# madeleineudell/LowRankModels.jl

Measured on AMD Instinct MI355X. Metric: observed-entry updates/sec, higher is better.
Workload: dtype f64

## Files before the change

lowrankmodels.jl_amd/csrc/glrm_cached.hpp:

```cpp
#pragma once

#include <hip/hip_runtime.h>

#include <algorithm>

#include "glrm_device.hpp"
#include "glrm_engine.hpp"
#include "glrm_launch.hpp"
#include "glrm_sweep.hpp"

namespace glrm {

struct CachedArgs {
  int64_t nseg;
  const int64_t* ptr;
  const int32_t* idx;
  const double* vals;
  double* own;
  int64_t own_offset;
  const double* other;
  double* alpha;
  const glrm_loss* losses;
  const glrm_reg* regs;
  int reg_single;
  int k;
  double fixed_alpha;
  double min_stepsize;
  int32_t* trials;
  int32_t* accepts;
  int cap;
  const int32_t* seglist;
  int64_t seg_lo, seg_hi;
  int vecreg;
};

__device__ __forceinline__ int64_t cached_segment(const CachedArgs& a, int64_t slot) {
  if (slot >= a.nseg) return -1;
  if (!a.seglist) return slot;
  const int64_t seg = a.seglist[slot];
  return (seg < a.seg_lo || seg >= a.seg_hi) ? -1 : seg;
}

__device__ __forceinline__ double cached_wide(double v) { return v; }
__device__ __forceinline__ double cached_wide(float v) {
  double d;
  asm volatile("v_cvt_f64_f32 %0, %1" : "=v"(d) : "v"(v));
  return d;
}

template <int G, int R, int LOSS, int MAXT, bool GRAD, int WAVES = 1, class ST = double>
__device__ __forceinline__ double reg_pass(const CachedArgs& a, const typename Pair<ST>::type (&y)[MAXT][R / 2], const ST (&av)[MAXT], const int (&cc)[MAXT],
                                           const Vec<G, R>& xv, Vec<G, R>& g, int len, int gi, const LossDesc& segloss) {
  constexpr int NG = (64 / G) * WAVES, LM = loss_mode(LOSS);
  constexpr bool TRIG = loss_trig(LOSS);
  double J = 0.0;
  if (GRAD) {
#pragma unroll
    for (int i = 0; i < R / 2; ++i) g.v[i] = make_double2(0.0, 0.0);
  }
#pragma unroll
  for (int t = 0; t < MAXT; ++t) {
    if (t * NG + (gi & ~(64 / G - 1)) < len) {
      double dot = 0.0;
#pragma unroll
      for (int i = 0; i < R / 2; ++i) {
        dot = fma(xv.v[i].x, cached_wide(y[t][i].x), dot);
        dot = fma(xv.v[i].y, cached_wide(y[t][i].y), dot);
      }
      dot = group_sum<G>(dot);
      double L, dL;
      if constexpr (LOSS == LOSS_QUAD_UNIFORM) {
        const double d = dot - (double)av[t];
        L = segloss.scale * (d * d);
        dL = 2 * d * segloss.scale;
      } else if constexpr (LM == LOSS_SEGMENT) {
        loss_both<GRAD, TRIG>(segloss, dot, (double)av[t], L, dL);
      } else {
        const LossDesc lo = load_loss(a.losses, cc[t]);
        loss_both<GRAD, TRIG>(lo, dot, (double)av[t], L, dL);
      }
      if (!(t * NG + gi < len)) {
        L = 0.0;
        dL = 0.0;
      }
      J += L;
      if (GRAD) {
#pragma unroll
        for (int i = 0; i < R / 2; ++i) {
          g.v[i].x = fma(dL, cached_wide(y[t][i].x), g.v[i].x);
          g.v[i].y = fma(dL, cached_wide(y[t][i].y), g.v[i].y);
        }
      }
    }
  }
  J = across_groups_sum<G>(J);
  if (GRAD) {
#pragma unroll
    for (int i = 0; i < R / 2; ++i) {
      g.v[i].x = across_groups_sum<G>(g.v[i].x);
      g.v[i].y = across_groups_sum<G>(g.v[i].y);
    }
  }
  return J;
}

template <int G, int R, int WAVES, bool GRAD>
__device__ __forceinline__ double row_combine(double J, Vec<G, R>& g, double* red, int wave, int lane) {
  constexpr int KP = G * R, STRIDE = KP + 2;
  if constexpr (WAVES == 1) return J;
  const int j = lane % G;
  __syncthreads();
  if (lane < G) {
    if (GRAD) {
#pragma unroll
      for (int i = 0; i < R / 2; ++i) *reinterpret_cast<double2*>(&red[wave * STRIDE + i * 2 * G + 2 * j]) = g.v[i];
    }
    if (lane == 0) red[wave * STRIDE + KP] = J;
  }
  __syncthreads();
  double Js = 0.0;
  if (GRAD) {
#pragma unroll
    for (int i = 0; i < R / 2; ++i) g.v[i] = make_double2(0.0, 0.0);
  }
  for (int w = 0; w < WAVES; ++w) {
    Js += red[w * STRIDE + KP];
    if (GRAD) {
#pragma unroll
      for (int i = 0; i < R / 2; ++i) {
        const double2 p = *reinterpret_cast<const double2*>(&red[w * STRIDE + i * 2 * G + 2 * j]);
        g.v[i].x += p.x;
        g.v[i].y += p.y;
      }
    }
  }
  return Js;
}

template <class ST, int G, int R>
__device__ __forceinline__ void round_trial(Vec<G, R>& xn) {
  if constexpr (sizeof(ST) == 4) {
#pragma unroll
    for (int i = 0; i < R / 2; ++i) xn.v[i] = make_double2(stored<ST>(xn.v[i].x), stored<ST>(xn.v[i].y));
  }
}

template <int G, int R, int LOSS, int MAXT, int WAVES, bool VR = false, class ST = double>
__global__ void __launch_bounds__(WAVES * 64) regcached_sweep_kernel(const CachedArgs a) {
  using P = typename Pair<ST>::type;
  constexpr int KP = G * R, NG = (64 / G) * WAVES;
  __shared__ __attribute__((aligned(16))) double red[WAVES == 1 ? 2 : WAVES * (KP + 2)];
  const int lane = threadIdx.x & 63, wave = threadIdx.x >> 6;
  const int64_t seg = cached_segment(a, blockIdx.x);
  if (seg < 0) return;
  const int j = lane % G, gi = wave * (64 / G) + lane / G;
  const int64_t beg = a.ptr[seg];
  const int len = (int)(a.ptr[seg + 1] - beg);
  const int64_t gseg = a.own_offset + seg;
  P* ownp = reinterpret_cast<P*>(reinterpret_cast<ST*>(a.own) + gseg * KP);
  const ST* vals = reinterpret_cast<const ST*>(a.vals);
  int cc[MAXT];
  ST av[MAXT];
  P y[MAXT][R / 2];
#pragma unroll
  for (int t = 0; t < MAXT; ++t) {
    int tt = t * NG + gi;
    tt = tt < len ? tt : (len > 0 ? len - 1 : 0);
    cc[t] = len > 0 ? a.idx[beg + tt] : 0;
    av[t] = len > 0 ? vals[beg + tt] : (ST)0.0;
  }
  Vec<G, R> x, g;
#pragma unroll
  for (int i = 0; i < R / 2; ++i) x.v[i] = widen(ownp[i * G + j]);
  const P* __restrict__ other2 = reinterpret_cast<const P*>(a.other);
#pragma unroll
  for (int t = 0; t < MAXT; ++t) {
    if (t * NG + wave * (64 / G) < len) {
      const P* yp = other2 + (int64_t)cc[t] * (KP / 2) + j;
#pragma unroll
      for (int i = 0; i < R / 2; ++i) y[t][i] = yp[i * G];
    } else {
#pragma unroll
      for (int i = 0; i < R / 2; ++i) y[t][i] = P{0, 0};
    }
  }
  const RegDesc rd = load_reg(a.regs, a.reg_single ? 0 : seg);
  LossDesc segloss = LossDesc{0, 1.0, 0.0, 0.0};
  if constexpr (loss_mode(LOSS) != LOSS_PER_OBS) segloss = load_loss(a.losses, 0);

  double Jold = reg_pass<G, R, LOSS, MAXT, true, WAVES, ST>(a, y, av, cc, x, g, len, gi, segloss);
  Jold = row_combine<G, R, WAVES, true>(Jold, g, red, wave, lane);
  if constexpr (sizeof(ST) == 8) {
    if (a.fixed_alpha > 0.0) {
      const double s = a.fixed_alpha / ((double)len + 1.0);
      Vec<G, R> xn;
#pragma unroll
      for (int i = 0; i < R / 2; ++i) {
        xn.v[i].x = x.v[i].x + g.v[i].x * (-s);
        xn.v[i].y = x.v[i].y + g.v[i].y * (-s);
      }
      reg_prox<G, R, VR>(rd, xn, s, j, a.k);
      if (gi == 0) {
#pragma unroll
        for (int i = 0; i < R / 2; ++i) store_pair<ST>(&ownp[i * G + j], xn.v[i]);
      }
      return;
    }
  }
  Jold += reg_eval<G, R, VR>(rd, x, j, a.k);
  double alpha = a.alpha[seg];
  const double l = (double)len + 1.0;
  int ntrials = 0;
  bool accepted = false;
  while (alpha > a.min_stepsize) {
    const double s = alpha / l;
    Vec<G, R> xn, dummy;
#pragma unroll
    for (int i = 0; i < R / 2; ++i) {
      xn.v[i].x = fma(-s, g.v[i].x, x.v[i].x);
      xn.v[i].y = fma(-s, g.v[i].y, x.v[i].y);
    }
    reg_prox<G, R, VR>(rd, xn, s, j, a.k);
    round_trial<ST>(xn);
    double Jn = reg_pass<G, R, LOSS, MAXT, false, WAVES, ST>(a, y, av, cc, xn, dummy, len, gi, segloss);
    Jn = row_combine<G, R, WAVES, false>(Jn, dummy, red, wave, lane);
    Jn += reg_eval<G, R, VR>(rd, xn, j, a.k);
    ++ntrials;
    if (Jn < Jold) {
      x = xn;
      alpha *= 1.05;
      Jold = Jn;
      accepted = true;
      break;
    }
    alpha *= .7;
    if (alpha < a.min_stepsize) {
      alpha = a.min_stepsize * 1.1;
      break;
    }
  }
  if (accepted && gi == 0) {
#pragma unroll
    for (int i = 0; i < R / 2; ++i) store_pair<ST>(&ownp[i * G + j], x.v[i]);
  }
  if (lane == 0 && wave == 0) {
    a.alpha[seg] = alpha;
    if (a.trials) {
      a.trials[seg] += ntrials;
      a.accepts[seg] += accepted ? 1 : 0;
    }
  }
}

template <class ST> constexpr int cached_persist_waves_per_simd() { return 2; }

template <int G, int R, int LOSS, int MAXT, bool VR = false, class ST = double>
__global__ void __launch_bounds__(128, cached_persist_waves_per_simd<ST>()) regcached_persist_kernel(const CachedArgs a) {
  using P = typename Pair<ST>::type;
  constexpr int WAVES = 2, KP = G * R, NG = (64 / G) * WAVES, MAXLEN = MAXT * NG, PF = (MAXLEN + 127) / 128;
  constexpr int VW = (int)sizeof(ST) / 4;
  constexpr int VALD = PF * 128 * VW / 2;
  constexpr int RED = WAVES * (KP + 2), REC = VALD + 128 + PF * 64;
  __shared__ __attribute__((aligned(16))) double sh[RED + 2 * REC];
  double* red = sh;
  const int tid = threadIdx.x, lane = tid & 63, wave = tid >> 6;
  const int j = lane % G, gi = wave * (64 / G) + lane / G;
  const RegDesc rd0 = load_reg(a.regs, 0);
  LossDesc segloss = LossDesc{0, 1.0, 0.0, 0.0};
  if constexpr (loss_mode(LOSS) != LOSS_PER_OBS) segloss = load_loss(a.losses, 0);
  const P* __restrict__ other2 = reinterpret_cast<const P*>(a.other);
  const ST* gvals = reinterpret_cast<const ST*>(a.vals);

  const auto* kptr = (const __attribute__((address_space(4))) int64_t*)a.ptr;
  const auto* klist = (const __attribute__((address_space(4))) int32_t*)a.seglist;
  auto seg_of = [&](int64_t slot) -> int64_t {
    if (slot >= a.nseg) return -1;
    if (!a.seglist) return slot;
    const int64_t s = klist[slot];
    return (s < a.seg_lo || s >= a.seg_hi) ? -1 : s;
  };
  auto rec_vals = [&](int buf) -> ST* { return reinterpret_cast<ST*>(sh + RED + buf * REC); };
  auto rec_alpha = [&](int buf) -> double* { return sh + RED + buf * REC + VALD; };
  auto rec_idx = [&](int buf) -> int* { return reinterpret_cast<int*>(sh + RED + buf * REC + VALD + 128); };
  auto fetch_rec = [&](int64_t sg, int64_t beg, int len, int (&pi)[PF], int (&pv)[VW * PF], double& pa) {
#pragma unroll
    for (int q = 0; q < PF; ++q) {
      int e = q * 128 + tid;
      e = e < len ? e : (len > 0 ? len - 1 : 0);
      pi[q] = len > 0 ? a.idx[beg + e] : 0;
      if constexpr (VW == 2) {
        const int2 v = len > 0 ? *reinterpret_cast<const int2*>(gvals + beg + e) : make_int2(0, 0);
        pv[2 * q] = v.x; pv[2 * q + 1] = v.y;
      } else {
        pv[q] = len > 0 ? *reinterpret_cast<const int*>(gvals + beg + e) : 0;
      }
    }
    pa = a.alpha[sg >= 0 ? sg : 0];
  };
  auto store_rec = [&](int buf, const int (&pi)[PF], const int (&pv)[VW * PF], double pa) {
    int* li = rec_idx(buf);
    int* lv = reinterpret_cast<int*>(rec_vals(buf));
#pragma unroll
    for (int q = 0; q < PF; ++q) {
      li[q * 128 + tid] = pi[q];
      if constexpr (VW == 2) {
        lv[2 * (q * 128 + tid)] = pv[2 * q];
        lv[2 * (q * 128 + tid) + 1] = pv[2 * q + 1];
      } else {
        lv[q * 128 + tid] = pv[q];
      }
    }
    rec_alpha(buf)[tid] = pa;
  };

  int64_t slot = blockIdx.x;
  int64_t seg = seg_of(slot), seg_n = seg_of(slot + gridDim.x);
  int64_t beg = seg >= 0 ? kptr[seg] : 0, beg_n = seg_n >= 0 ? kptr[seg_n] : 0;
  int len = seg >= 0 ? (int)(kptr[seg + 1] - beg) : 0, len_n = seg_n >= 0 ? (int)(kptr[seg_n + 1] - beg_n) : 0;
  {
    int pi[PF], pv[VW * PF];
    double pa;
    fetch_rec(seg, beg, len, pi, pv, pa);
    store_rec(0, pi, pv, pa);
  }
  __syncthreads();
  int cur = 0;
  for (; slot < a.nseg; slot += gridDim.x) {
    int64_t seg_nn, beg_nn;
    int len_nn;
    auto next_pointers = [&] {
      seg_nn = seg_of(slot + 2 * (int64_t)gridDim.x);
      const int64_t p0 = kptr[seg_nn >= 0 ? seg_nn : 0], p1 = kptr[(seg_nn >= 0 ? seg_nn : 0) + 1];
      beg_nn = seg_nn >= 0 ? p0 : 0;
      len_nn = seg_nn >= 0 ? (int)(p1 - p0) : 0;
    };
    if (seg < 0) {
      int pi[PF], pv[VW * PF];
      double pa;
      fetch_rec(seg_n, beg_n, len_n, pi, pv, pa);
      next_pointers();
      store_rec(cur ^ 1, pi, pv, pa);
    } else {
      const ST* lvals = rec_vals(cur);
      const int* lidx = rec_idx(cur);
      int cc[MAXT];
      ST av[MAXT];
      P y[MAXT][R / 2];
#pragma unroll
      for (int t = 0; t < MAXT; ++t) {
        int tt = t * NG + gi;
        tt = tt < len ? tt : (len > 0 ? len - 1 : 0);
        cc[t] = lidx[tt];
        av[t] = lvals[tt];
      }
      const int64_t gseg = a.own_offset + seg;
      P* ownp = reinterpret_cast<P*>(reinterpret_cast<ST*>(a.own) + gseg * KP);
      Vec<G, R> x, g;
#pragma unroll
      for (int i = 0; i < R / 2; ++i) x.v[i] = widen(ownp[i * G + j]);
#pragma unroll
      for (int t = 0; t < MAXT; ++t) {
        if (t * NG + wave * (64 / G) < len) {
          const P* yp = other2 + (int64_t)cc[t] * (KP / 2) + j;
#pragma unroll
          for (int i = 0; i < R / 2; ++i) y[t][i] = yp[i * G];
        } else {
#pragma unroll
          for (int i = 0; i < R / 2; ++i) y[t][i] = P{0, 0};
        }
      }
      int pi[PF], pv[VW * PF];
      double pa;
      fetch_rec(seg_n, beg_n, len_n, pi, pv, pa);
      next_pointers();
      const RegDesc rd = a.reg_single ? rd0 : load_reg(a.regs, seg);

      double Jold = reg_pass<G, R, LOSS, MAXT, true, WAVES, ST>(a, y, av, cc, x, g, len, gi, segloss);
      Jold = row_combine<G, R, WAVES, true>(Jold, g, red, wave, lane);
      store_rec(cur ^ 1, pi, pv, pa);
      bool fixed = false;
      if constexpr (sizeof(ST) == 8) fixed = a.fixed_alpha > 0.0;
      if (fixed) {
        const double s = a.fixed_alpha / ((double)len + 1.0);
        Vec<G, R> xn;
#pragma unroll
        for (int i = 0; i < R / 2; ++i) {
          xn.v[i].x = x.v[i].x + g.v[i].x * (-s);
          xn.v[i].y = x.v[i].y + g.v[i].y * (-s);
        }
        reg_prox<G, R, VR>(rd, xn, s, j, a.k);
        if (gi == 0) {
#pragma unroll
          for (int i = 0; i < R / 2; ++i) store_pair<ST>(&ownp[i * G + j], xn.v[i]);
        }
      } else {
        Jold += reg_eval<G, R, VR>(rd, x, j, a.k);
        double alpha = rec_alpha(cur)[tid];
        const double l = (double)len + 1.0;
        int ntrials = 0;
        bool accepted = false;
        while (alpha > a.min_stepsize) {
          const double s = alpha / l;
          Vec<G, R> xn, dummy;
#pragma unroll
          for (int i = 0; i < R / 2; ++i) {
            xn.v[i].x = fma(-s, g.v[i].x, x.v[i].x);
            xn.v[i].y = fma(-s, g.v[i].y, x.v[i].y);
          }
          reg_prox<G, R, VR>(rd, xn, s, j, a.k);
          round_trial<ST>(xn);
          double Jn = reg_pass<G, R, LOSS, MAXT, false, WAVES, ST>(a, y, av, cc, xn, dummy, len, gi, segloss);
          Jn = row_combine<G, R, WAVES, false>(Jn, dummy, red, wave, lane);
          Jn += reg_eval<G, R, VR>(rd, xn, j, a.k);
          ++ntrials;
          if (Jn < Jold) {
            x = xn;
            alpha *= 1.05;
            Jold = Jn;
            accepted = true;
            break;
          }
          alpha *= .7;
          if (alpha < a.min_stepsize) {
            alpha = a.min_stepsize * 1.1;
            break;
          }
        }
        if (accepted && gi == 0) {
#pragma unroll
          for (int i = 0; i < R / 2; ++i) store_pair<ST>(&ownp[i * G + j], x.v[i]);
        }
        if (tid == 0) {
          a.alpha[seg] = alpha;
          if (a.trials) {
            atomicAdd(&a.trials[seg], ntrials);
            atomicAdd(&a.accepts[seg], accepted ? 1 : 0);
          }
        }
      }
    }
    __syncthreads();
    cur ^= 1;
    seg = seg_n; beg = beg_n; len = len_n;
    seg_n = seg_nn; beg_n = beg_nn; len_n = len_nn;
  }
}

template <int G, int R, int LOSS, bool VR, class ST = double>
int launch_reg_inst(const CachedArgs& a, hipStream_t st, glrm_handle* h) {
  constexpr bool F32 = sizeof(ST) == 4;
  const int waves = F32 ? 2 : env_int("GLRM_HIP_CACHED_WAVES", 2);
  if (waves == 2 && env_int("GLRM_HIP_CACHED_PERSIST", 1)) {
    const bool small = (a.cap + 1) / 2 <= 4;
    int& cache = h->cached_grid[(small ? 1 : 0) + (VR ? 2 : 0) + (F32 ? 4 : 0)];
    int nb = cache;
    if (nb == 0) {
      int per_cu = 0;
      hipDeviceProp_t prop;
      const void* k = small ? (const void*)regcached_persist_kernel<G, R, LOSS, 4, VR, ST> : (const void*)regcached_persist_kernel<G, R, LOSS, 7, VR, ST>;
      if (hipOccupancyMaxActiveBlocksPerMultiprocessor(&per_cu, k, 128, 0) != hipSuccess || per_cu < 1) { (void)hipGetLastError(); per_cu = 1; }
      int cus = 256;
      if (hipGetDeviceProperties(&prop, h->device) == hipSuccess && prop.multiProcessorCount > 0) cus = prop.multiProcessorCount;
      nb = per_cu * cus;
      if (nb < 1) nb = 1;
      cache = nb;
    }
    const unsigned grid = (unsigned)std::min<int64_t>(a.nseg, nb);
    if (small) hipLaunchKernelGGL((regcached_persist_kernel<G, R, LOSS, 4, VR, ST>), dim3(grid), dim3(128), 0, st, a);
    else hipLaunchKernelGGL((regcached_persist_kernel<G, R, LOSS, 7, VR, ST>), dim3(grid), dim3(128), 0, st, a);
    return GLRM_OK;
  }
  if constexpr (!F32) {
    if (waves == 4 && (a.cap + 3) / 4 <= 4) {
      hipLaunchKernelGGL((regcached_sweep_kernel<G, R, LOSS, 4, 4, VR, ST>), dim3((unsigned)a.nseg), dim3(256), 0, st, a);
      return GLRM_OK;
    }
    if (waves == 1) {
      if (a.cap <= 7) hipLaunchKernelGGL((regcached_sweep_kernel<G, R, LOSS, 7, 1, VR, ST>), dim3((unsigned)a.nseg), dim3(64), 0, st, a);
      else hipLaunchKernelGGL((regcached_sweep_kernel<G, R, LOSS, 13, 1, VR, ST>), dim3((unsigned)a.nseg), dim3(64), 0, st, a);
      return GLRM_OK;
    }
  }
  if ((a.cap + 1) / 2 <= 4) {
    hipLaunchKernelGGL((regcached_sweep_kernel<G, R, LOSS, 4, 2, VR, ST>), dim3((unsigned)a.nseg), dim3(128), 0, st, a);
  } else {
    hipLaunchKernelGGL((regcached_sweep_kernel<G, R, LOSS, 7, 2, VR, ST>), dim3((unsigned)a.nseg), dim3(128), 0, st, a);
  }
  return GLRM_OK;
}

}

int glrm_launch_cached_f32(const glrm::CachedArgs& a, int G, int loss, hipStream_t st, glrm_handle* h);
```

Before: 11.19 billion.

## Add triple-buffered persistent kernel using global-to-LDS DMA record prefetch

Adds a new f64 persistent kernel that prefetches each segment's indices, values, own row and alpha two segments ahead into a triple-buffered LDS ring. It uses inline-asm global_load_lds_dword so the copies go straight to shared memory without passing through registers. Output writes are deferred and flushed at the start of the next iteration so they overlap the following segment. The kernel is on by default through GLRM_HIP_CACHED_STAGE. In exchange it uses more LDS, which can lower occupancy, and relies on fragile inline asm that manages m0 and vmcnt by hand.

Result: no change. 11.27 billion, median of 6 (+0.8%).

```diff
diff --git a/lowrankmodels.jl_amd/csrc/glrm_cached.hpp b/lowrankmodels.jl_amd/csrc/glrm_cached.hpp
--- a/lowrankmodels.jl_amd/csrc/glrm_cached.hpp
+++ b/lowrankmodels.jl_amd/csrc/glrm_cached.hpp
@@ -446,18 +446,239 @@
   }
 }
 
+__device__ __forceinline__ void record_dma(const void* gsrc, unsigned lds_dst) {
+  unsigned keep;
+  asm volatile("s_mov_b32 %0, m0\n\ts_mov_b32 m0, %2\n\ts_nop 0\n\tglobal_load_lds_dword %1, off\n\ts_mov_b32 m0, %0"
+               : "=&s"(keep) : "v"(gsrc), "s"(lds_dst) : "memory");
+}
+
+template <int G, int R, int LOSS, int MAXT, bool VR>
+__global__ void __launch_bounds__(128, 2) regcached_persist_kernel_ahead(const CachedArgs a) {
+  using ST = double;
+  using P = double2;
+  constexpr int WAVES = 2, KP = G * R, NG = (64 / G) * WAVES, MAXLEN = MAXT * NG, PF = (MAXLEN + 127) / 128;
+  constexpr int VALD = PF * 128, RED = WAVES * (KP + 2), REC = VALD + 32 + 64 + PF * 64;
+  __shared__ __attribute__((aligned(16))) double sh[RED + 3 * REC];
+  double* red = sh;
+  const int tid = threadIdx.x, lane = tid & 63, wave = tid >> 6;
+  const int j = lane % G, gi = wave * (64 / G) + lane / G;
+  const int wv = __builtin_amdgcn_readfirstlane(wave);
+  const RegDesc rd0 = load_reg(a.regs, 0);
+  LossDesc segloss = LossDesc{0, 1.0, 0.0, 0.0};
+  if constexpr (loss_mode(LOSS) != LOSS_PER_OBS) segloss = load_loss(a.losses, 0);
+  const P* __restrict__ other2 = reinterpret_cast<const P*>(a.other);
+  const ST* gvals = reinterpret_cast<const ST*>(a.vals);
+  const auto* kptr = (const __attribute__((address_space(4))) int64_t*)a.ptr;
+  const auto* klist = (const __attribute__((address_space(4))) int32_t*)a.seglist;
+  auto seg_of = [&](int64_t slot) -> int64_t {
+    if (slot >= a.nseg) return -1;
+    if (!a.seglist) return slot;
+    const int64_t s = klist[slot];
+    return (s < a.seg_lo || s >= a.seg_hi) ? -1 : s;
+  };
+  auto rec_vals = [&](int buf) -> ST* { return sh + RED + buf * REC; };
+  auto rec_alpha = [&](int buf) -> double* { return sh + RED + buf * REC + VALD; };
+  auto rec_x = [&](int buf) -> double* { return sh + RED + buf * REC + VALD + 32; };
+  auto rec_idx = [&](int buf) -> int* { return reinterpret_cast<int*>(sh + RED + buf * REC + VALD + 96); };
+  auto lds_of = [&](const void* p) -> unsigned { return (unsigned)(uintptr_t)(__attribute__((address_space(3))) const void*)p; };
+  const unsigned sh_lds = lds_of(sh);
+  auto lane_now = [] {
+    int l;
+    asm volatile("v_mbcnt_lo_u32_b32 %0, -1, 0\n\tv_mbcnt_hi_u32_b32 %0, -1, %0" : "=v"(l));
+    return l;
+  };
+  auto rec_issue = [&](int buf, int64_t sg, int64_t beg_, int len_) {
+    const unsigned base = sh_lds + (unsigned)((RED + buf * REC) * 8);
+    const int lane = lane_now(), tid = wv * 64 + lane;
+    if (len_ > 0) {
+#pragma unroll
+      for (int q = 0; q < PF; ++q) {
+        int e = q * 128 + tid;
+        e = e < len_ ? e : len_ - 1;
+        record_dma(a.idx + beg_ + e, base + (unsigned)((VALD + 96) * 8 + (q * 128 + wv * 64) * 4));
+#pragma unroll
+        for (int r = 0; r < 2; ++r) {
+          const int d = r * 128 + tid;
+          int ev = q * 128 + d / 2;
+          ev = ev < len_ ? ev : len_ - 1;
+          record_dma(reinterpret_cast<const int*>(gvals + beg_ + ev) + (d & 1), base + (unsigned)((q * 256 + r * 128 + wv * 64) * 4));
+        }
+      }
+    }
+    record_dma(reinterpret_cast<const int*>(a.own + (a.own_offset + sg) * KP) + tid % (2 * KP), base + (unsigned)((VALD + 32) * 8 + wv * 256));
+    if (wv == 0) record_dma(reinterpret_cast<const int*>(a.alpha + sg) + (lane & 1), base + (unsigned)(VALD * 8));
+  };
+
+  const int64_t grid = gridDim.x;
+  int64_t slot = blockIdx.x;
+  int64_t seg = seg_of(slot), seg_n = seg_of(slot + grid);
+  int len, len_n;
+  {
+    const int64_t beg = seg >= 0 ? kptr[seg] : 0, beg_n = seg_n >= 0 ? kptr[seg_n] : 0;
+    len = seg >= 0 ? (int)(kptr[seg + 1] - beg) : 0;
+    len_n = seg_n >= 0 ? (int)(kptr[seg_n + 1] - beg_n) : 0;
+    if (seg >= 0) rec_issue(0, seg, beg, len);
+    if (seg_n >= 0) rec_issue(1, seg_n, beg_n, len_n);
+  }
+  asm volatile("s_waitcnt vmcnt(0)" ::: "memory");
+  __syncthreads();
+  int cur = 0;
+  Vec<G, R> xo;
+#pragma unroll
+  for (int i = 0; i < R / 2; ++i) xo.v[i] = make_double2(0.0, 0.0);
+  bool out_x = false, out_a = false;
+  int out_alpha_lo = 0, out_alpha_hi = 0, out_trials = 0, out_accepts = 0;
+  int64_t out_seg = 0;
+  auto flush_out = [&] {
+    const int lane = lane_now();
+    if (out_x) {
+      P* op = reinterpret_cast<P*>(a.own + (a.own_offset + out_seg) * KP);
+#pragma unroll
+      for (int i = 0; i < R / 2; ++i) op[i * G + lane % G] = xo.v[i];
+    }
+    if (out_a && wv == 0 && lane == 0) {
+      a.alpha[out_seg] = __hiloint2double(out_alpha_hi, out_alpha_lo);
+      if (a.trials) {
+        atomicAdd(&a.trials[out_seg], out_trials);
+        atomicAdd(&a.accepts[out_seg], out_accepts);
+      }
+    }
+    out_x = out_a = false;
+  };
+  for (; slot < a.nseg; slot += grid) {
+    const int nxt = cur == 2 ? 0 : cur + 1, nn = nxt == 2 ? 0 : nxt + 1;
+    int64_t seg_nn, beg_nn;
+    int len_nn;
+    auto next_pointers = [&] {
+      seg_nn = seg_of(slot + 2 * grid);
+      const int64_t p0 = kptr[seg_nn >= 0 ? seg_nn : 0], p1 = kptr[(seg_nn >= 0 ? seg_nn : 0) + 1];
+      beg_nn = seg_nn >= 0 ? p0 : 0;
+      len_nn = seg_nn >= 0 ? (int)(p1 - p0) : 0;
+    };
+    auto request_record = [&] {
+      if (seg_nn >= 0) rec_issue(nn, seg_nn, beg_nn, len_nn);
+    };
+    asm volatile("s_waitcnt vmcnt(0)" ::: "memory");
+    flush_out();
+    if (seg < 0) {
+      next_pointers();
+      request_record();
+    } else {
+      const ST* lvals = rec_vals(cur);
+      const int* lidx = rec_idx(cur);
+      int cc[MAXT];
+      ST av[MAXT];
+      P y[MAXT][R / 2];
+#pragma unroll
+      for (int t = 0; t < MAXT; ++t) {
+        int tt = t * NG + gi;
+        tt = tt < len ? tt : (len > 0 ? len - 1 : 0);
+        cc[t] = lidx[tt];
+        av[t] = lvals[tt];
+      }
+      Vec<G, R> x, g;
+#pragma unroll
+      for (int i = 0; i < R / 2; ++i) x.v[i] = *reinterpret_cast<const double2*>(&rec_x(cur)[2 * (i * G + j)]);
+#pragma unroll
+      for (int t = 0; t < MAXT; ++t) {
+        if (t * NG + wave * (64 / G) < len) {
+          const P* yp = other2 + (int64_t)cc[t] * (KP / 2) + j;
+#pragma unroll
+          for (int i = 0; i < R / 2; ++i) y[t][i] = yp[i * G];
+        } else {
+#pragma unroll
+          for (int i = 0; i < R / 2; ++i) y[t][i] = P{0, 0};
+        }
+      }
+      next_pointers();
+      const RegDesc rd = a.reg_single ? rd0 : load_reg(a.regs, seg);
+
+      double Jold = reg_pass<G, R, LOSS, MAXT, true, WAVES, ST>(a, y, av, cc, x, g, len, gi, segloss);
+      asm volatile("" ::"v"(rd.kind), "v"(rd.scale));
+#pragma unroll
+      for (int t = 0; t < MAXT; ++t) {
+#pragma unroll
+        for (int i = 0; i < R / 2; ++i) asm volatile("" ::"v"(y[t][i].x), "v"(y[t][i].y));
+      }
+      request_record();
+      Jold = row_combine<G, R, WAVES, true>(Jold, g, red, wave, lane);
+      out_seg = seg;
+      if (a.fixed_alpha > 0.0) {
+        const double s = a.fixed_alpha / ((double)len + 1.0);
+#pragma unroll
+        for (int i = 0; i < R / 2; ++i) {
+          xo.v[i].x = x.v[i].x + g.v[i].x * (-s);
+          xo.v[i].y = x.v[i].y + g.v[i].y * (-s);
+        }
+        reg_prox<G, R, VR>(rd, xo, s, j, a.k);
+        out_x = gi == 0;
+      } else {
+        Jold += reg_eval<G, R, VR>(rd, x, j, a.k);
+        double alpha = rec_alpha(cur)[0];
+        const double l = (double)len + 1.0;
+        int ntrials = 0;
+        bool accepted = false;
+        while (alpha > a.min_stepsize) {
+          const double s = alpha / l;
+          Vec<G, R> xn, dummy;
+#pragma unroll
+          for (int i = 0; i < R / 2; ++i) {
+            xn.v[i].x = fma(-s, g.v[i].x, x.v[i].x);
+            xn.v[i].y = fma(-s, g.v[i].y, x.v[i].y);
+          }
+          reg_prox<G, R, VR>(rd, xn, s, j, a.k);
+          double Jn = reg_pass<G, R, LOSS, MAXT, false, WAVES, ST>(a, y, av, cc, xn, dummy, len, gi, segloss);
+          Jn = row_combine<G, R, WAVES, false>(Jn, dummy, red, wave, lane);
+          Jn += reg_eval<G, R, VR>(rd, xn, j, a.k);
+          ++ntrials;
+          if (Jn < Jold) {
+            x = xn;
+            alpha *= 1.05;
+            Jold = Jn;
+            accepted = true;
+            break;
+          }
+          alpha *= .7;
+          if (alpha < a.min_stepsize) {
+            alpha = a.min_stepsize * 1.1;
+            break;
+          }
+        }
+        xo = x;
+        out_x = accepted && gi == 0;
+        out_a = true;
+        out_alpha_lo = __builtin_amdgcn_readfirstlane(__double2loint(alpha));
+        out_alpha_hi = __builtin_amdgcn_readfirstlane(__double2hiint(alpha));
+        out_trials = __builtin_amdgcn_readfirstlane(ntrials);
+        out_accepts = __builtin_amdgcn_readfirstlane(accepted ? 1 : 0);
+      }
+    }
+    __syncthreads();
+    cur = nxt;
+    seg = seg_n; len = len_n;
+    seg_n = seg_nn; len_n = len_nn;
+  }
+  asm volatile("s_waitcnt vmcnt(0)" ::: "memory");
+  flush_out();
+}
+
 template <int G, int R, int LOSS, bool VR, class ST = double>
 int launch_reg_inst(const CachedArgs& a, hipStream_t st, glrm_handle* h) {
   constexpr bool F32 = sizeof(ST) == 4;
   const int waves = F32 ? 2 : env_int("GLRM_HIP_CACHED_WAVES", 2);
   if (waves == 2 && env_int("GLRM_HIP_CACHED_PERSIST", 1)) {
     const bool small = (a.cap + 1) / 2 <= 4;
+    bool staged = false;
+    if constexpr (!F32) staged = env_int("GLRM_HIP_CACHED_STAGE", 1) != 0;
     int& cache = h->cached_grid[(small ? 1 : 0) + (VR ? 2 : 0) + (F32 ? 4 : 0)];
     int nb = cache;
     if (nb == 0) {
       int per_cu = 0;
       hipDeviceProp_t prop;
       const void* k = small ? (const void*)regcached_persist_kernel<G, R, LOSS, 4, VR, ST> : (const void*)regcached_persist_kernel<G, R, LOSS, 7, VR, ST>;
+      if constexpr (!F32) {
+        if (staged) k = small ? (const void*)regcached_persist_kernel_ahead<G, R, LOSS, 4, VR> : (const void*)regcached_persist_kernel_ahead<G, R, LOSS, 7, VR>;
+      }
       if (hipOccupancyMaxActiveBlocksPerMultiprocessor(&per_cu, k, 128, 0) != hipSuccess || per_cu < 1) { (void)hipGetLastError(); per_cu = 1; }
       int cus = 256;
       if (hipGetDeviceProperties(&prop, h->device) == hipSuccess && prop.multiProcessorCount > 0) cus = prop.multiProcessorCount;
@@ -466,6 +687,13 @@
       cache = nb;
     }
     const unsigned grid = (unsigned)std::min<int64_t>(a.nseg, nb);
+    if constexpr (!F32) {
+      if (staged) {
+        if (small) hipLaunchKernelGGL((regcached_persist_kernel_ahead<G, R, LOSS, 4, VR>), dim3(grid), dim3(128), 0, st, a);
+        else hipLaunchKernelGGL((regcached_persist_kernel_ahead<G, R, LOSS, 7, VR>), dim3(grid), dim3(128), 0, st, a);
+        return GLRM_OK;
+      }
+    }
     if (small) hipLaunchKernelGGL((regcached_persist_kernel<G, R, LOSS, 4, VR, ST>), dim3(grid), dim3(128), 0, st, a);
     else hipLaunchKernelGGL((regcached_persist_kernel<G, R, LOSS, 7, VR, ST>), dim3(grid), dim3(128), 0, st, a);
     return GLRM_OK;
```
